# bkomuves/zikkurat-algebra

Hardware: AMD Instinct MI355X
Metric: BLS12-381 G1 MSM pairs/sec at 2^20; Fr NTT 2^24 elems/sec (1/2/4/8 GPU) (higher is better)
Workload: dtype u32-limb Montgomery Fp (381-bit)

## Files before the change

zikkurat-algebra_amd/csrc/zk_hostpool.cpp:

```cpp
#include <atomic>
#include <condition_variable>
#include <functional>
#include <memory>
#include <mutex>
#include <thread>
#include <vector>
#include "zk_hostpool.hpp"

namespace zk {

namespace {
struct Job {
  const std::function<void(int)> *fn;
  int n;
  std::atomic<int> next{0}, done{0};
  Job(const std::function<void(int)> *f, int count) : fn(f), n(count) {}
  bool has_work() const { return next.load(std::memory_order_relaxed) < n; }
  void drain() {
    for (;;) {
      const int i = next.fetch_add(1);
      if (i >= n) break;
      (*fn)(i);
      done.fetch_add(1, std::memory_order_release);
    }
  }
};

struct HostPool {
  std::mutex mu;
  std::condition_variable cv;
  std::vector<std::shared_ptr<Job>> active;
  int workers = 0;
  HostPool() {
    unsigned hw = std::thread::hardware_concurrency();
    workers = hw > 2 ? (int)(hw - 1 < 7 ? hw - 1 : 7) : 0;
    for (int i = 0; i < workers; i++) std::thread([this] { loop(); }).detach();
  }
  std::shared_ptr<Job> pick() {
    for (auto &j : active)
      if (j->has_work()) return j;
    return nullptr;
  }
  void loop() {
    for (;;) {
      std::shared_ptr<Job> job;
      {
        std::unique_lock<std::mutex> lk(mu);
        cv.wait(lk, [&] { return (job = pick()) != nullptr; });
      }
      job->drain();
    }
  }
  void run(int count, const std::function<void(int)> &f, const std::function<void()> *main_fn = nullptr) {
    auto job = std::make_shared<Job>(&f, count);
    {
      std::lock_guard<std::mutex> lk(mu);
      active.push_back(job);
    }
    cv.notify_all();
    if (main_fn) (*main_fn)();
    job->drain();
    while (job->done.load(std::memory_order_acquire) < count) std::this_thread::yield();
    std::lock_guard<std::mutex> lk(mu);
    for (size_t i = 0; i < active.size(); i++)
      if (active[i] == job) {
        active.erase(active.begin() + i);
        break;
      }
  }
};
}

static HostPool *shared_pool() {
  static HostPool *pool = new HostPool();
  return pool;
}

void host_parallel_for(int n, const std::function<void(int)> &fn) {
  if (n <= 0) return;
  HostPool *pool = shared_pool();
  if (n == 1 || pool->workers == 0) {
    for (int i = 0; i < n; i++) fn(i);
    return;
  }
  pool->run(n, fn);
}

void host_parallel_for_main(int n, const std::function<void(int)> &fn, const std::function<void()> &main_fn) {
  HostPool *pool = shared_pool();
  if (n <= 0 || pool->workers == 0) {
    for (int i = 0; i < n; i++) fn(i);
    main_fn();
    return;
  }
  pool->run(n, fn, &main_fn);
}

}
```

zikkurat-algebra_amd/csrc/zk_hostpool.hpp:

```cpp
#pragma once
#include <functional>

namespace zk {

void host_parallel_for(int n, const std::function<void(int)> &fn);

void host_parallel_for_main(int n, const std::function<void(int)> &fn, const std::function<void()> &main_fn);

}
```

zikkurat-algebra_amd/csrc/zk_msm_impl.hpp:

```cpp
#pragma once
#include <hipcub/hipcub.hpp>
#include <algorithm>
#include <atomic>
#include <chrono>
#include <memory>
#include <thread>
#include <vector>
#include "zk_curve.hpp"
#include "zk_quad.hpp"
#include "zk_host.hpp"
#include "zk_runtime.hpp"
#include "zk_msm.hpp"
#include "zk_ntt.hpp"

namespace zk {

template <class C>
__global__ void __launch_bounds__(256) k_points_int(const uint64_t *__restrict__ pts, int n,
                                                    uint32_t *__restrict__ out) {
  using F = typename C::Fp;
  constexpr int IN4 = 2 * F::N64 * 8 / 16;
  constexpr int OUT4 = aff_words<F>() / 4;
  constexpr int ST4 = IN4 > OUT4 ? IN4 : OUT4;
  __shared__ uint4 stage[256 * ST4];
// ... 473 lines not shown
        if (first_run && bbeg < cs) {
          xyzz_store(ivals + (size_t)(2 * t) * xyzz_words<F>(), acc);
          k0 = b;
        } else {
          xyzz_store(buckets + (size_t)b * xyzz_words<F>(), acc);
        }
        first_run = false;
        do {
          b++;
          bbeg = bend;
          bend = bnext;
          bnext = offsets[min(b + 2, nb)];
        } while (bend <= e);
        start_run(b);
      }
      if (P.x.v[0] != 0xffffffffu) {
        if (c0 & 0x80000000u) {
          Fe<F> ny;
          fe_neg(ny, P.y);
          P.y = ny;
        }
        xyzz_acc_aff(acc, P);
      }
      c0 = c1;
      c1 = c2;
    }
    const bool lpart = bbeg < cs, rpart = bend > ce;
    if (rpart && !(first_run && lpart)) {
      tail_b = b;
      tail_slot = first_run ? 2 * t : 2 * t + 1;
    } else if (lpart || rpart) {
      xyzz_store(ivals + (size_t)(2 * t) * xyzz_words<F>(), acc);
      k0 = b;
    } else {
      xyzz_store(buckets + (size_t)b * xyzz_words<F>(), acc);
    }
    head_end = k0 != nb && !(first_run && rpart);
    asm volatile("s_waitcnt vmcnt(0)" ::: "memory");
  }
  __builtin_amdgcn_fence(__ATOMIC_RELEASE, "workgroup");
  const uint32_t nhead = (uint32_t)__shfl_down((int)(head_end ? k0 : nb), 1, 64);
  const bool merge = tail_b != nb && lane < 63 && nhead == tail_b;
  if (__any(merge)) {
    __builtin_amdgcn_fence(__ATOMIC_ACQUIRE, "workgroup");
    if (merge) {
      const uint32_t *src = ivals + (size_t)(2 * t + 2) * xyzz_words<F>();
      uint32_t wds[xyzz_words<F>()];
#pragma unroll
      for (int i = 0; i < xyzz_words<F>(); i++) wds[i] = __hip_atomic_load(src + i, __ATOMIC_RELAXED, __HIP_MEMORY_SCOPE_AGENT);
      Xyzz<F> o;
      xyzz_load(o, wds);
      xyzz_add(acc, o);
    }
  }
  if (tail_b != nb) {
    if (merge) {
      xyzz_store(buckets + (size_t)tail_b * xyzz_words<F>(), acc);
    } else {
      xyzz_store(ivals + (size_t)tail_slot * xyzz_words<F>(), acc);
      if (tail_slot == 2 * t) k0 = tail_b; else k1 = tail_b;
    }
  }
  if (__shfl_up((int)merge, 1, 64) && lane > 0) k0 = nb;
  if (2 * t < nslots) {
    ikeys[2 * t] = k0;
    ikeys[2 * t + 1] = k1;
  }
}

static __global__ void __launch_bounds__(256) k_fill_mark(const uint32_t *__restrict__ off, uint32_t nb, int first,
                                                          uint8_t *__restrict__ filled) {
  const uint32_t b = blockIdx.x * blockDim.x + threadIdx.x;
  if (b >= nb) return;
  const uint8_t f = off[b + 1] > off[b] ? 1 : 0;
  filled[b] = first ? f : (uint8_t)(filled[b] | f);
}

static __global__ void __launch_bounds__(256) k_item_flags(const uint32_t *__restrict__ ikeys, const uint32_t *__restrict__ count,
                                                    uint32_t nslots_max, uint32_t nb, uint32_t *__restrict__ flags) {
  const uint32_t i = blockIdx.x * blockDim.x + threadIdx.x;
  if (i >= nslots_max) return;
  const uint32_t n = count ? *count : nslots_max;
  flags[i] = (i < n && ikeys[i] < nb) ? 1u : 0u;
}
#ifndef ZK_STITCH_RAW
#define ZK_STITCH_RAW 1
#endif
template <class C, int BS>
__global__ void __launch_bounds__(BS) k_stitch_blk(const uint32_t *__restrict__ keys, const uint32_t *__restrict__ idx,
                                                   const uint32_t *__restrict__ vals,
                                                   const uint32_t *__restrict__ count, uint32_t nb, uint32_t W,
                                                   uint32_t B, uint32_t *__restrict__ buckets,
                                                   uint32_t *__restrict__ okeys, uint32_t *__restrict__ ovals,
                                                   uint32_t nout) {
  using F = typename C::Fp;
  constexpr int XW = xyzz_words<F>();
  __shared__ uint4 stitch_lds4[BS * XW / 4];
  uint32_t *lv = reinterpret_cast<uint32_t *>(stitch_lds4);
  __shared__ uint32_t skey[BS];
  const uint32_t M = *count;
  const uint32_t t = threadIdx.x, blk = blockIdx.x;
  const uint32_t base = blk * BS;
  if (base >= M) {
    if (t < 2 && 2 * blk + t < nout) okeys[2 * blk + t] = nb;
    return;
  }
  const uint32_t nv = min((uint32_t)BS, M - base);
  const uint32_t j = base + t;
  const bool valid = t < nv;
  const uint32_t key = valid ? keys[j] : 0xffffffffu;
  skey[t] = key;
  Xyzz<F> acc;
  if (valid) xyzz_load(acc, vals + (size_t)idx[j] * XW);
  else xyzz_set_inf(acc);
  __syncthreads();
  for (uint32_t d = 1; d < nv; d <<= 1) {
    const bool need = valid && t >= d && skey[t - d] == key;
    if (!__syncthreads_or(need)) break;
    xyzz_store(lv + (size_t)t * XW, acc);
    __syncthreads();
    if (need) {
      Xyzz<F> o;
      xyzz_load(o, lv + (size_t)(t - d) * XW);
      xyzz_add_red(acc, o);
    }
    __syncthreads();
  }
  if (!valid) return;
  const bool seg_last = t == nv - 1 || skey[t + 1] != key;
  if (!seg_last) return;
  const bool touches_start = skey[0] == key;
  const bool touches_end = t == nv - 1;
  const bool cont_in = touches_start && base > 0 && keys[base - 1] == key;
  const bool cont_out = touches_end && base + nv < M && keys[base + nv] == key;
  if (!cont_in && !cont_out) {
    xyzz_store(buckets + (size_t)key * XW, acc);
  } else {
    xyzz_store(ovals + (size_t)(touches_start ? 2 * blk : 2 * blk + 1) * XW, acc);
  }
  const uint32_t item_key = (cont_in || cont_out) ? key : nb;
  if (touches_start) okeys[2 * blk] = item_key;
  if (touches_end) okeys[2 * blk + 1] = touches_start ? nb : item_key;
}

#ifndef ZK_STITCH_QUAD
#define ZK_STITCH_QUAD 1
#endif
constexpr int STITCH_QBS = 64;
template <class C>
__global__ void __launch_bounds__(256) k_stitch_blk_q(const uint32_t *__restrict__ keys, const uint32_t *__restrict__ idx,
                                                      const uint32_t *__restrict__ vals,
                                                      const uint32_t *__restrict__ count, uint32_t nb,
                                                      uint32_t *__restrict__ buckets, uint32_t *__restrict__ okeys,
                                                      uint32_t *__restrict__ ovals, uint32_t nout) {
  using F = typename C::Fp;
  constexpr int XW = xyzz_words<F>();
  constexpr uint32_t BSQ = STITCH_QBS;
  __shared__ uint4 item_lds4[BSQ * XW / 4];
  __shared__ uint32_t skey[BSQ];
  uint32_t *lv = reinterpret_cast<uint32_t *>(item_lds4);
  uint32_t *const park = nullptr;
  const uint32_t M = *count;
  const uint32_t tq = threadIdx.x >> 2, q = threadIdx.x & 3, blk = blockIdx.x;
  const uint32_t base = blk * BSQ;
  if (base >= M) {
    if (threadIdx.x < 2 && 2 * blk + threadIdx.x < nout) okeys[2 * blk + threadIdx.x] = nb;
// ... 728 lines not shown
    add(maxent * 2);
    add((s.nmat2() + 1) * 4 * 2);
  }
  add(s.NS * (nb + 1) * 4);
  add(nb);
  add(ns0 * (xw + 4) + ns0 * 16 + 64);
  add(ns1 * (xw + 4) * 2);
  add(nb * xw);
  add((size_t)s.W * s.NY * xw);
  add(cub > cub2 ? cub : cub2);
  if (s.NS > 1) add(cub > cub2 ? cub : cub2);
  return bytes + (1 << 20);
}

inline std::atomic<int> &msm_last_groups() {
  static std::atomic<int> v{0};
  return v;
}

inline std::atomic<int> &msm_profile_flag() {
  static std::atomic<int> on{0};
  return on;
}
struct PhaseProf {
  bool on = false;
  hipStream_t st = nullptr;
  std::vector<std::pair<const char *, hipEvent_t>> ev;
  explicit PhaseProf(hipStream_t s) : st(s) {
    on = msm_profile_flag().load() != 0;
    mark("start");
  }
  void mark(const char *name) {
    if (!on) return;
    hipEvent_t e;
    ZK_CHECK(hipEventCreate(&e));
    ZK_CHECK(hipEventRecord(e, st));
    ev.emplace_back(name, e);
  }
  void report(double host_ms) {
    if (!on) return;
    ZK_CHECK(hipStreamSynchronize(st));
    fprintf(stderr, "[zk msm]");
    for (size_t i = 1; i < ev.size(); i++) {
      float ms = 0;
      ZK_CHECK(hipEventElapsedTime(&ms, ev[i - 1].second, ev[i].second));
      fprintf(stderr, " %s=%.3f", ev[i].first, ms);
    }
    fprintf(stderr, " host_finish=%.3f ms\n", host_ms);
    for (auto &e : ev) ZK_CHECK(hipEventDestroy(e.second));
    ev.clear();
  }
};

struct ScalarSlice {
  const uint64_t *data;
  int stride, loff, nread;
  bool mont;
};

template <class C>
struct GroupPass {
  using F = typename C::Fp;
  static constexpr int STITCH_BS = stitch_bs<F>();
  Device &dev;
  MsmShape s;
  ScalarSlice sc;
  int wbase, timer_slot;
  const uint32_t *pts_int;
  uint64_t *h;
  PhaseProf *prof;
  hipStream_t st;
  size_t nb, xw, maxent, ns0, ns1, cub = 0;
  uint32_t *list, *dig, *tmpv, *cnt, *coff, *offsets, *ikeys0, *ivals0, *ckeys, *cidx, *flags, *pos, *ccount;
  uint16_t *tmpf, *tmpf2 = nullptr;
  uint32_t *cnt2 = nullptr, *coff2 = nullptr;
  uint32_t *okA, *ovA, *okB, *ovB, *buckets, *Y;
  void *cubtmp;
  uint8_t *filled = nullptr;
  hipStream_t sst = nullptr;
  void *cubtmp_sort = nullptr;
  const uint64_t *pts_ref = nullptr;
  std::vector<hipEvent_t> sorted_ev;
  hipEvent_t presorted = nullptr;
  const uint32_t *inK, *inV;
  size_t slots;
  uint32_t *outK, *outV, *altK, *altV;

  GroupPass(Device &d, const MsmShape &shape, const ScalarSlice &scal, int wb, const uint32_t *pts, uint64_t *hh,
            PhaseProf *pr, hipStream_t stream, int tslot)
      : dev(d), s(shape), sc(scal), wbase(wb), timer_slot(tslot), pts_int(pts), h(hh), prof(pr), st(stream) {
    const int n = s.n;
    nb = (size_t)s.W * s.B;
    xw = xyzz_words<F>();
    maxent = (size_t)s.W * n;
    ZK_REQUIRE(maxent <= MSM_MAX_PASS_ENTRIES, "msm: window group exceeds the sort capacity (internal sizing bug)");
    list = dev.arena.take<uint32_t>(maxent);
    dig = dev.arena.take<uint32_t>(maxent);
    tmpv = dev.arena.take<uint32_t>(maxent);
    tmpf = dev.arena.take<uint16_t>(maxent);
    cnt = dev.arena.take<uint32_t>(s.nmat() + 1);
    coff = dev.arena.take<uint32_t>(s.nmat() + 1);
    if (s.s2) {
      tmpf2 = dev.arena.take<uint16_t>(maxent);
      cnt2 = dev.arena.take<uint32_t>(s.nmat2() + 1);
      coff2 = dev.arena.take<uint32_t>(s.nmat2() + 1);
    }
    offsets = dev.arena.take<uint32_t>((size_t)s.NS * (nb + 1));
    if (s.NS > 1) filled = dev.arena.take<uint8_t>(nb);
    ns0 = stitch_slots0(s);
    ns1 = stitch_slots1(s, stitch_bs0<F>());
    ikeys0 = dev.arena.take<uint32_t>(ns0);
    ivals0 = dev.arena.take<uint32_t>(ns0 * xw);
    ckeys = dev.arena.take<uint32_t>(ns0);
    cidx = dev.arena.take<uint32_t>(ns0);
    flags = dev.arena.take<uint32_t>(ns0);
    pos = dev.arena.take<uint32_t>(ns0);
    ccount = dev.arena.take<uint32_t>(16);
    okA = dev.arena.take<uint32_t>(ns1);
    ovA = dev.arena.take<uint32_t>(ns1 * xw);
    okB = dev.arena.take<uint32_t>(ns1);
    ovB = dev.arena.take<uint32_t>(ns1 * xw);
    buckets = dev.arena.take<uint32_t>(nb * xw);
    Y = dev.arena.take<uint32_t>((size_t)s.W * s.NY * xw);
    size_t cub2 = 0;
    ZK_CHECK(hipcub::DeviceScan::ExclusiveSum(nullptr, cub, cnt, coff, (int)(s.nmat() + 1), st));
    ZK_CHECK(hipcub::DeviceScan::ExclusiveSum(nullptr, cub2, flags, pos, (int)ns0, st));
    if (cub2 > cub) cub = cub2;
    if (s.s2) {
      size_t cub3 = 0;
      ZK_CHECK(hipcub::DeviceScan::ExclusiveSum(nullptr, cub3, cnt2, coff2, (int)(s.nmat2() + 1), st));
      if (cub3 > cub) cub = cub3;
    }
    cubtmp = dev.arena.take<char>(cub);
    if (s.NS > 1) cubtmp_sort = dev.arena.take<char>(cub);
  }
  void mark(const char *what) {
    if (prof && wbase == 0) prof->mark(what);
  }

  void sort(int sp, hipStream_t st, void *cubtmp) {
    const int n = s.n, c = s.c;
    const int lo = s.split_lo(sp), hi = s.split_lo(sp + 1);
    const uint32_t base = (uint32_t)((size_t)s.W * lo);
    hipLaunchKernelGGL(k_digits<C>, dim3(div_up(hi - lo, 256)), dim3(256), 0, st, sc.data, n, lo, hi, sc.stride,
                       sc.loff, sc.nread, sc.mont ? 1 : 0, c, wbase, s.W, dig);
    ZK_CHECK(hipGetLastError());
    if (st == this->st) mark("digits");
    const dim3 grid((unsigned)s.nwg, (unsigned)s.W);
    hipLaunchKernelGGL(k_coarse<false>, grid, dim3(256), 0, st, dig, n, lo, hi, s.M, s.fs, s.nbins, cnt, tmpv + base,
                       tmpf + base);
    ZK_CHECK(hipGetLastError());
    size_t cb = cub;
    ZK_CHECK(hipcub::DeviceScan::ExclusiveSum(cubtmp, cb, cnt, coff, (int)(s.nmat() + 1), st));
    hipLaunchKernelGGL(k_coarse<true>, grid, dim3(256), 0, st, dig, n, lo, hi, s.M, s.fs, s.nbins, coff, tmpv + base,
                       tmpf + base);
    ZK_CHECK(hipGetLastError());
    const uint32_t *fv = tmpv + base, *fcoff = coff;
    const uint16_t *ff = tmpf + base;
    int fnwg = s.nwg, fs = s.fs;
    uint32_t nq = (uint32_t)(s.W * s.nbins);
    if (s.s2) {
      const int nsub = 1 << s.s2, s2sh = s.fs - s.s2;
      const dim3 g2((unsigned)s.nwg2, nq);
      hipLaunchKernelGGL(k_split<false>, g2, dim3(256), 0, st, coff, s.nwg, s2sh, nsub, cnt2, tmpv + base, tmpf + base,
                         dig + base, tmpf2 + base);
      ZK_CHECK(hipGetLastError());
      size_t cb2 = cub;
      ZK_CHECK(hipcub::DeviceScan::ExclusiveSum(cubtmp, cb2, cnt2, coff2, (int)(s.nmat2() + 1), st));
      hipLaunchKernelGGL(k_split<true>, g2, dim3(256), 0, st, coff, s.nwg, s2sh, nsub, coff2, tmpv + base, tmpf + base,
                         dig + base, tmpf2 + base);
      ZK_CHECK(hipGetLastError());
      fv = dig + base;
      ff = tmpf2 + base;
      fcoff = coff2;
      fnwg = s.nwg2;
      fs = s2sh;
      nq *= (uint32_t)nsub;
    }
    const int cap = fine_stage_cap(fs);
    const int lds = (4 << fs) + 4 * cap;
    if ((size_t)(hi - lo) * s.W >= (size_t)nq * 4096) {
      ZK_CHECK(hipFuncSetAttribute((const void *)k_fine<1024, 4, true>, hipFuncAttributeMaxDynamicSharedMemorySize,
                                   lds));
      hipLaunchKernelGGL((k_fine<1024, 4, true>), dim3(nq), dim3(1024), lds, st, fcoff, fnwg, nq, fs, cap, fv, ff,
                         list + base, offsets + (size_t)sp * (nb + 1), base);
    } else {
      ZK_CHECK(hipFuncSetAttribute((const void *)k_fine<256, 1, false>, hipFuncAttributeMaxDynamicSharedMemorySize,
                                   lds));
      hipLaunchKernelGGL((k_fine<256, 1, false>), dim3(nq), dim3(256), lds, st, fcoff, fnwg, nq, fs, cap, fv, ff,
                         list + base, offsets + (size_t)sp * (nb + 1), base);
    }
    ZK_CHECK(hipGetLastError());
    if (st == this->st) mark("sort");
  }

  std::vector<hipEvent_t> wait_sc, wait_pt;
  const std::atomic<int> *ready_sc = nullptr, *ready_pt = nullptr;
  void wait_for(hipStream_t on, const std::vector<hipEvent_t> &ev, const std::atomic<int> *ready, int sp) {
    if (sp >= (int)ev.size() || !ev[sp]) return;
    if (ready)
      while (!ready[sp].load(std::memory_order_acquire)) std::this_thread::yield();
    ZK_CHECK(hipStreamWaitEvent(on, ev[sp], 0));
  }
  void convert(int sp) {
    const int lo = s.split_lo(sp), hi = s.split_lo(sp + 1);
    if (hi <= lo) return;
    hipLaunchKernelGGL(k_points_int<C>, dim3(div_up(hi - lo, 256)), dim3(256), 0, st,
                       pts_ref + (size_t)lo * 2 * C::NP64, hi - lo, const_cast<uint32_t *>(pts_int) + (size_t)lo * aff_words<F>());
    ZK_CHECK(hipGetLastError());
  }
  int ch0 = 0;
  void accumulate(int sp) {
    if (sp == 0) timer_begin(dev, timer_slot, st);
    const size_t npts = (size_t)s.split_lo(sp + 1) - (size_t)s.split_lo(sp);
    const int CH = s.split_ch(sp);
    ch0 = CH;
    const size_t nsl = 2 * (((size_t)s.W * npts + CH - 1) / CH);
    hipLaunchKernelGGL(k_accum<C>, dim3(div_up(nsl / 2, 256)), dim3(256), 0, st, pts_int, list,
                       offsets + (size_t)sp * (nb + 1), (uint32_t)nb, CH, (uint32_t)s.W, (uint32_t)s.B, buckets,
                       ikeys0, ivals0, (uint32_t)nsl, (const uint8_t *)(sp > 0 ? filled : nullptr));
    ZK_CHECK(hipGetLastError());
    if (sp == s.NS - 1) timer_end(dev, timer_slot, st);
    mark("accum");
    inK = ikeys0;
    inV = ivals0;
    slots = nsl;
    level = 0;
    outK = okA; outV = ovA; altK = okB; altV = ovB;
  }
  void fill_mark(int sp) {
    hipLaunchKernelGGL(k_fill_mark, dim3(div_up(nb, 256)), dim3(256), 0, st, offsets + (size_t)sp * (nb + 1),
                       (uint32_t)nb, sp == 0 ? 1 : 0, filled);
    ZK_CHECK(hipGetLastError());
  }

  int level = 0;
  bool stitch_level() {
    const bool raw = ZK_STITCH_RAW && level++ > 0;
    const bool quad0 = stitch_bs0<F>() == STITCH_QBS && (ns0 <= 65536 || ch0 >= 64);
    const int bs = raw ? STITCH_BS : (quad0 ? STITCH_QBS : STITCH_BS);
    const bool final_level = slots <= (size_t)bs;
    const size_t nout = final_level ? 2 : 2 * ((slots + bs - 1) / bs);
    if (raw) {
      hipLaunchKernelGGL((k_stitch_raw<C, STITCH_BS>), dim3((unsigned)((slots + STITCH_BS - 1) / STITCH_BS)),
                         dim3(STITCH_BS), 0, st, inK, inV, (uint32_t)slots, (uint32_t)nb, final_level ? 1 : 0,
                         buckets, outK, outV);
      ZK_CHECK(hipGetLastError());
    } else {
      hipLaunchKernelGGL(k_item_flags, dim3(div_up(slots, 256)), dim3(256), 0, st, inK, (const uint32_t *)nullptr,
                         (uint32_t)slots, (uint32_t)nb, flags);
      ZK_CHECK(hipGetLastError());
      size_t cb = cub;
      ZK_CHECK(hipcub::DeviceScan::ExclusiveSum(cubtmp, cb, flags, pos, (int)slots, st));
      hipLaunchKernelGGL(k_item_index, dim3(div_up(slots, 256)), dim3(256), 0, st, inK, flags, pos, (uint32_t)slots,
                         ckeys, cidx, ccount);
      ZK_CHECK(hipGetLastError());
      bool launched = false;
      if constexpr (stitch_bs0<F>() == STITCH_QBS) {
        if (quad0) {
          hipLaunchKernelGGL(k_stitch_blk_q<C>, dim3((unsigned)(nout / 2)), dim3(256), 0, st, ckeys, cidx, inV, ccount,
                             (uint32_t)nb, buckets, outK, outV, (uint32_t)nout);
          launched = true;
        }
      }
      if (!launched)
        hipLaunchKernelGGL((k_stitch_blk<C, STITCH_BS>), dim3((unsigned)(nout / 2)), dim3(STITCH_BS), 0, st, ckeys,
                           cidx, inV, ccount, (uint32_t)nb, (uint32_t)s.W, (uint32_t)s.B, buckets, outK, outV,
                           (uint32_t)nout);
      ZK_CHECK(hipGetLastError());
    }
    inK = outK; inV = outV; slots = nout;
    uint32_t *tk = outK, *tv = outV;
    outK = altK; outV = altV; altK = tk; altV = tv;
    return final_level;
  }

  void reduce_tail() {
    const int c = s.c;
    const int n0 = s.r0.count * s.r0.G, n1 = s.r1.count * s.r1.G;
    if (n0 % 256 == 0 && n1 % 256 == 0) {
      const unsigned nblk = (unsigned)(s.W * (n0 + n1) / 256);
      bool two_waves = false;
      if constexpr (is_base_field<F>()) {
        two_waves = ysum3_on((size_t)nblk * 256);
        if (two_waves)
          hipLaunchKernelGGL((k_ysum3<C>), dim3(nblk), dim3(256), 0, st, buckets, offsets, (const uint8_t *)filled,
                             s.W, c, s.l0, s.r0, s.r1, Y);
      } else if (ysum_g2_lds<F>()) {
        two_waves = true;
        hipLaunchKernelGGL((k_ysum3<C, 1>), dim3(nblk), dim3(256), 0, st, buckets, offsets, (const uint8_t *)filled,
                           s.W, c, s.l0, s.r0, s.r1, Y);
      }
      if (!two_waves)
        hipLaunchKernelGGL((k_ysum2<C, is_base_field<F>() ? ZK_YSUM_PF != 0 : ZK_YSUM_PF_G2 != 0>), dim3(nblk),
                           dim3(256), 0, st, buckets, offsets,
                           (const uint8_t *)filled, s.W, c, s.l0, s.r0, s.r1, Y);
    } else {
      const size_t lanes = (size_t)s.W * s.ylanes;
      hipLaunchKernelGGL(k_ysum<C>, dim3(div_up(lanes, 256)), dim3(256), 0, st, buckets, offsets,
                         (const uint8_t *)filled, s.W, c, s.l0, s.r0, s.r1, s.ylanes, Y);
    }
    ZK_CHECK(hipGetLastError());
    mark("ysum");
    hipLaunchKernelGGL(k_jobsum_blk<C>, dim3((unsigned)(s.W * c)), dim3(256), 0, st, Y, c, s.l0, h);
    ZK_CHECK(hipGetLastError());
    mark("jobsum");
  }

  void launch() {
    for (int sp = 0; sp < s.NS; sp++) {
      if (presorted) {
        ZK_CHECK(hipStreamWaitEvent(st, presorted, 0));
      } else if (sst) {
        wait_for(sst, wait_sc, ready_sc, sp);
        sort(sp, sst, cubtmp_sort);
        ZK_CHECK(hipEventRecord(sorted_ev[sp], sst));
      } else {
        wait_for(st, wait_sc, ready_sc, sp);
        sort(sp, st, cubtmp);
      }
      wait_for(st, wait_pt, ready_pt, sp);
      if (pts_ref) convert(sp);
      if (sst) ZK_CHECK(hipStreamWaitEvent(st, sorted_ev[sp], 0));
      accumulate(sp);
      for (bool final_level = false; !final_level;) final_level = stitch_level();
      if (s.NS > 1) fill_mark(sp);
    }
    mark("stitch");
    reduce_tail();
  }
  void finish() {
    stream_wait(dev, st);
    mark("export");
  }
};

template <class C>
static void finish_host(int c, int W, const uint64_t *exported, zkh::Xyzz<typename HostOf<C>::Fp> &out,
                        int bits = 0) {
  using HF = typename HostOf<C>::Fp;
  const int NP = C::NP64;
  const int J = c, E = bits ? c : c - 1;
  std::vector<zkh::Jac<HF>> V(W);
  std::unique_ptr<std::atomic<int>[]> ready(new std::atomic<int>[W]);
  for (int w = 0; w < W; w++) ready[w].store(0, std::memory_order_relaxed);
  std::atomic<int> next_win{0};
  auto window = [&](int i) {
    const int w = W - 1 - i;
    std::vector<zkh::Xyzz<HF>> Z(E);
    for (auto &z : Z) zkh::xyzz_set_inf(z);
    for (int j = 0; j < J; j++) {
      if (bits && c * w + j >= bits) break;
      const uint64_t *q = exported + ((size_t)w * J + j) * 4 * NP;
      zkh::Xyzz<HF> p;
      memcpy(p.X.v, q + 0 * NP, NP * 8);
      memcpy(p.Y.v, q + 1 * NP, NP * 8);
      memcpy(p.ZZ.v, q + 2 * NP, NP * 8);
      memcpy(p.ZZZ.v, q + 3 * NP, NP * 8);
      if (zkh::xyzz_is_inf(p)) continue;
      const int e = bits ? j : (j == 0 ? 0 : j - 1);
      zkh::xyzz_add(Z[e], Z[e], p);
    }
    zkh::Xyzz<HF> acc;
    zkh::xyzz_set_inf(acc);
    for (int e = E - 1; e >= 0; e--) {
      zkh::xyzz_dbl(acc, acc);
      zkh::xyzz_add(acc, acc, Z[e]);
    }
    zkh::xyzz_to_jac(V[w], acc);
    ready[w].store(1, std::memory_order_release);
  };
  zkh::Jac<HF> acc;
  zkh::jac_set_inf(acc);
  auto claim = [&]() -> bool {
    const int i = next_win.fetch_add(1);
    if (i >= W) return false;
    window(i);
    return true;
  };
  auto chain = [&] {
    for (int w = W - 1; w >= 0; w--) {
      for (int k = 0; k < c; k++) zkh::jac_dbl(acc, acc);
      while (!ready[w].load(std::memory_order_acquire))
        if (!claim()) std::this_thread::yield();
      zkh::jac_add(acc, acc, V[w]);
    }
  };
  const int nthreads = W < 8 ? W : 8;
  host_parallel_for_main(nthreads, [&](int) { while (claim()) {} }, chain);
  zkh::jac_to_xyzz(out, acc);
}

#ifndef ZK_MSM_BITS_MAX
#define ZK_MSM_BITS_MAX 4096
#endif
inline int msm_bits_max() {
  static const int v = [] {
    const char *e = getenv("ZK_MSM_BITS_MAX");
    return e ? atoi(e) : ZK_MSM_BITS_MAX;
  }();
  return v;
}
inline int msm_bits_groups(int n) {
  static const int g = [] {
    const char *e = getenv("ZK_MSM_BITS_G");
    const int v = e ? atoi(e) : 256;
    return v >= 1 ? v : 256;
  }();
  int K = (n + g - 1) / g;
  if (K > BITACC_MAX_K) K = BITACC_MAX_K;
  return (n + K - 1) / K;
}

template <class C>
static void msm_run_bits(Device &dev, int n, const ScalarSlice &sc_in, const uint64_t *points, bool host_inputs,
                         int nbits, zkh::Xyzz<typename HostOf<C>::Fp> &out) {
  using F = typename C::Fp;
  constexpr int XW = xyzz_words<F>();
  ZK_REQUIRE(nbits >= 1 && nbits <= 256, "msm: bit-job path takes at most 256-bit scalars (internal)");
  const int G = msm_bits_groups(n), K = (n + G - 1) / G;
  ZK_REQUIRE(K >= 1 && K <= BITACC_MAX_K, "msm: bit-job chunk larger than k_bitacc's LDS staging (internal)");
  hipStream_t st = dev.stream;
  const size_t sc_bytes = host_inputs ? (size_t)n * sc_in.stride * 8 : 0;
  const size_t pt_bytes = host_inputs ? (size_t)n * 2 * C::NP64 * 8 : 0;
  const size_t int_bytes = (size_t)n * aff_words<F>() * 4;
  const size_t part_bytes = (size_t)nbits * G * XW * 4;
  const size_t exp_bytes = (size_t)nbits * 4 * C::NP64 * 8;
  const size_t need = sc_bytes + pt_bytes + int_bytes + part_bytes + 4 * 256;
  if (!dev.arena.try_reserve(need)) {
    ZK_CHECK(hipStreamSynchronize(st));
    ntt_release(dev);
    ZK_REQUIRE(dev.arena.try_reserve(need), "msm: out of device memory");
  }
  dev.arena.reset();
  msm_last_groups().store(1);
  PhaseProf prof(st);
  ScalarSlice sc = sc_in;
  const uint64_t *pts_ref = points;
  if (host_inputs) {
    uint64_t *a = dev.arena.take<uint64_t>((size_t)n * sc_in.stride);
    uint64_t *b = dev.arena.take<uint64_t>((size_t)n * 2 * C::NP64);
    ZK_CHECK(hipMemcpyAsync(a, sc_in.data, sc_bytes, hipMemcpyHostToDevice, st));
    ZK_CHECK(hipMemcpyAsync(b, points, pt_bytes, hipMemcpyHostToDevice, st));
    sc.data = a;
    pts_ref = b;
  }
  uint32_t *pts_int = dev.arena.take<uint32_t>((size_t)n * aff_words<F>());
  uint32_t *part = dev.arena.take<uint32_t>((size_t)nbits * G * XW);
  uint64_t *h = reinterpret_cast<uint64_t *>(dev.host_staging(exp_bytes + 64));
  hipLaunchKernelGGL(k_points_int<C>, dim3(div_up(n, 256)), dim3(256), 0, st, pts_ref, n, pts_int);
  ZK_CHECK(hipGetLastError());
  prof.mark("points");
  timer_begin(dev, 0, st);
  hipLaunchKernelGGL(k_bitacc<C>, dim3((unsigned)G), dim3(256), 0, st, sc.data, n, sc.stride, sc.loff, sc.nread,
                     sc.mont ? 1 : 0, nbits, K, pts_int, part);
  ZK_CHECK(hipGetLastError());
  timer_end(dev, 0, st);
  prof.mark("bitacc");
  hipLaunchKernelGGL(k_bitsum<C>, dim3((unsigned)nbits), dim3(256), 0, st, part, G, h);
  ZK_CHECK(hipGetLastError());
  prof.mark("bitsum");
  stream_wait(dev, st);
  prof.mark("export");
  timer_collect(dev);
  const auto t0 = std::chrono::steady_clock::now();
  constexpr int BW = 8;
  finish_host<C>(BW, (nbits + BW - 1) / BW, h, out, nbits);
// ... 51 lines not shown
                                           group_bytes<C>(make_shape(n, c, W - Wa, 1)));
  while (!ahead && !dev.arena.try_reserve(sc_bytes + pt_bytes + int_bytes + 3 * 256 + group_bytes<C>(s))) {
    if (!dropped_twiddles) {
      ZK_CHECK(hipStreamSynchronize(st));
      ntt_release(dev);
      dropped_twiddles = true;
      continue;
    }
    ZK_REQUIRE(Wg > 1, "msm: out of device memory (one window per pass does not fit)");
    Wg = (Wg + 1) / 2;
    s = make_shape(n, c, Wg, splits(Wg));
  }
  const int NS = s.NS;
  msm_last_groups().store(ahead ? 2 : (W + Wg - 1) / Wg);
  dev.arena.reset();
  ScalarSlice sc = sc_in;
  uint32_t *pts_int = nullptr;
  PhaseProf prof(st);
  bool inputs_on_aux = false;
  std::atomic<int> ready_sc[ZK_MSM_SPLITS_MAX], ready_pt[ZK_MSM_SPLITS_MAX];
  std::string copy_err;
  std::mutex copy_mu;
  std::vector<std::thread> copier_v;
  JoinAll join_copier{copier_v};
  uint64_t *pts_ref = nullptr;
  if (host_inputs) {
    uint64_t *a = dev.arena.take<uint64_t>((size_t)n * sc_in.stride);
    uint64_t *b = dev.arena.take<uint64_t>((size_t)n * 2 * C::NP64);
    pts_int = dev.arena.take<uint32_t>((size_t)n * aff_words<F>());
    sc.data = a;
    pts_ref = b;
    hipStream_t st2 = dev.aux_stream();
    for (int h = 0; h < 3 * NS; h++) dev.split_event(h);
    for (int h = 0; h < NS; h++) {
      ready_sc[h].store(0, std::memory_order_relaxed);
      ready_pt[h].store(0, std::memory_order_relaxed);
    }
    const int stride = sc_in.stride;
    const uint64_t *sc_host = sc_in.data;
    const MsmShape shp = s;
    copier_v.emplace_back([&dev, st2, NS, shp, a, b, stride, sc_host, points, &ready_sc, &ready_pt, &copy_err,
                           &copy_mu] {
      catch_into(&copy_err, &copy_mu, [&] {
      ZK_CHECK(hipSetDevice(dev.id));
      for (int h = 0; h < NS; h++) {
        const int lo = shp.split_lo(h), hi = shp.split_lo(h + 1);
        ZK_CHECK(hipMemcpyAsync(a + (size_t)lo * stride, sc_host + (size_t)lo * stride,
                                (size_t)(hi - lo) * stride * 8, hipMemcpyHostToDevice, st2));
        ZK_CHECK(hipEventRecord(dev.split_event(3 * h), st2));
        ready_sc[h].store(1, std::memory_order_release);
        const size_t off = (size_t)lo * 2 * C::NP64;
        ZK_CHECK(hipMemcpyAsync(b + off, points + off, (size_t)(hi - lo) * 2 * C::NP64 * 8, hipMemcpyHostToDevice, st2));
        ZK_CHECK(hipEventRecord(dev.split_event(3 * h + 1), st2));
        ready_pt[h].store(1, std::memory_order_release);
      }
      });
      for (int h = 0; h < NS; h++) {
        ready_sc[h].store(1, std::memory_order_release);
        ready_pt[h].store(1, std::memory_order_release);
      }
    });
    inputs_on_aux = true;
  } else {
    pts_int = dev.arena.take<uint32_t>((size_t)n * aff_words<F>());
    if (ahead) ZK_CHECK(hipEventRecord(dev.split_event(0), st));
    hipLaunchKernelGGL(k_points_int<C>, dim3(div_up(n, 256)), dim3(256), 0, st, points, n, pts_int);
    ZK_CHECK(hipGetLastError());
  }
  prof.mark("points");
  const size_t mark = dev.arena.used();
  const size_t per_w = (size_t)c * 4 * C::NP64;
  uint64_t *h = reinterpret_cast<uint64_t *>(dev.host_staging((size_t)W * per_w * 8 + 64));
  if (ahead) {
    GroupPass<C> pa(dev, make_shape(n, c, Wa, 1), sc, 0, pts_int, h, &prof, st, 0);
    GroupPass<C> pb(dev, make_shape(n, c, W - Wa, 1), sc, Wa, pts_int, h + (size_t)Wa * per_w, &prof, st, 1);
    hipStream_t sst = dev.aux2_stream();
    ZK_CHECK(hipStreamWaitEvent(sst, dev.split_event(0), 0));
    pa.sort(0, sst, pa.cubtmp);
    ZK_CHECK(hipEventRecord(dev.split_event(1), sst));
    pb.sort(0, sst, pb.cubtmp);
    ZK_CHECK(hipEventRecord(dev.split_event(2), sst));
    pa.presorted = dev.split_event(1);
    pb.presorted = dev.split_event(2);
    pa.launch();
    pb.launch();
    pb.finish();
    timer_collect(dev);
    const auto t0 = std::chrono::steady_clock::now();
    finish_host<C>(c, W, h, out);
    prof.report(std::chrono::duration<double, std::milli>(std::chrono::steady_clock::now() - t0).count());
    return;
  }
  for (int wbase = 0; wbase < W; wbase += Wg) {
    dev.arena.rewind(mark);
    const MsmShape sg = (wbase + Wg <= W) ? s : make_shape(n, c, W - wbase);
    GroupPass<C> pass(dev, sg, sc, wbase, pts_int, h + (size_t)wbase * per_w, &prof, st, wbase == 0 ? 0 : -1);
    if (inputs_on_aux) {
      ZK_REQUIRE(sg.NS == NS, "msm: split pipeline shape mismatch (internal)");
      for (int h = 0; h < NS; h++) {
        pass.wait_sc.push_back(dev.split_event(3 * h));
        pass.wait_pt.push_back(dev.split_event(3 * h + 1));
        pass.sorted_ev.push_back(dev.split_event(3 * h + 2));
      }
      pass.ready_sc = ready_sc;
      pass.ready_pt = ready_pt;
      pass.pts_ref = pts_ref;
      static const bool sort_inline = [] {
        const char *e = getenv("ZK_MSM_SORT_INLINE");
        return e && e[0] == '1';
      }();
      if (NS > 1 && !sort_inline) pass.sst = dev.aux2_stream();
    }
    inputs_on_aux = false;
    pass.launch();
    for (auto &t : copier_v)
      if (t.joinable()) t.join();
    pass.finish();
    rethrow_first(copy_err);
  }
  timer_collect(dev);
  const auto t0 = std::chrono::steady_clock::now();
  finish_host<C>(c, W, h, out);
  prof.report(std::chrono::duration<double, std::milli>(std::chrono::steady_clock::now() - t0).count());
}


template <class C>
size_t msm_workspace_bytes(int n, int nl, bool mont, bool host_inputs, int window, int groups) {
  using F = typename C::Fp;
  if (n <= 0) return 0;
  const int nread = nl < 4 ? nl : 4;
  const int nbits = mont ? HostOf<C>::Fr::BITS : 64 * nread;
  if (!(window >= 4 && window <= 24) && n <= msm_bits_max()) {
    const size_t io = host_inputs ? (size_t)n * nl * 8 + (size_t)n * 2 * C::NP64 * 8 : 0;
    return io + (size_t)n * aff_words<F>() * 4 + (size_t)nbits * msm_bits_groups(n) * xyzz_words<F>() * 4 + 4 * 256;
  }
  const int c = (window >= 4 && window <= 24)
                    ? window
                    : (is_base_field<F>() ? msm_default_window_bits(n, nbits) : msm_default_window(n));
  const int W = nbits / c + 1;
  const int g = groups < 1 ? 1 : (groups > W ? W : groups);
  const int Wg = (W + g - 1) / g;
  const size_t sc_bytes = host_inputs ? (size_t)n * nl * 8 : 0;
  const size_t pt_bytes = host_inputs ? (size_t)n * 2 * C::NP64 * 8 : 0;
  const size_t int_bytes = (size_t)n * aff_words<F>() * 4;
  const int NS = msm_splits(n, host_inputs, Wg == W);
  if (msm_ahead<C>(n, host_inputs, W, Wg)) {
    const int Wa = (W + 1) / 2;
    return int_bytes + 3 * 256 + group_bytes<C>(make_shape(n, c, Wa, 1)) + group_bytes<C>(make_shape(n, c, W - Wa, 1));
  }
  return sc_bytes + pt_bytes + int_bytes + 3 * 256 + group_bytes<C>(make_shape(n, c, Wg, NS));
}

template <class C>
static void msm_xyzz(Device &dev, int n, const uint64_t *scalars, int nl, const uint64_t *points, bool host_inputs,
                     bool mont, int window, zkh::Xyzz<typename HostOf<C>::Fp> &acc) {
  using HF = typename HostOf<C>::Fp;
  if (mont || nl <= 4) {
    msm_run<C>(dev, n, ScalarSlice{scalars, nl, 0, nl < 4 ? nl : 4, mont}, points, host_inputs, window, acc);
  } else {
    zkh::xyzz_set_inf(acc);
    const int nsl = (nl + 3) / 4;
    for (int j = nsl - 1; j >= 0; j--) {
      for (int k = 0; k < 256; k++) zkh::xyzz_dbl(acc, acc);
      const int nread = nl - 4 * j < 4 ? nl - 4 * j : 4;
      zkh::Xyzz<HF> r;
      msm_run<C>(dev, n, ScalarSlice{scalars, nl, 4 * j, nread, false}, points, host_inputs, window, r);
      zkh::xyzz_add(acc, acc, r);
    }
  }
}

template <class C>
void msm_g1(int n, const uint64_t *scalars, int nl, const uint64_t *points, bool host_inputs, bool mont,
            int window, uint64_t *out_proj) {
  using HF = typename HostOf<C>::Fp;
  ZK_REQUIRE(nl >= 1, "msm: expo_nlimbs must be >= 1");
  zkh::Xyzz<HF> acc;
  const std::vector<int> set = host_inputs ? device_set() : std::vector<int>();
  const int G = (int)set.size();
  if (G > 1 && n > 0) {
    std::vector<zkh::Xyzz<HF>> part(G);
    std::vector<std::thread> th;
    std::string err;
    std::mutex emu;
    {
    JoinAll join_all{th};
    for (int k = 0; k < G; k++) {
      const size_t lo = (size_t)n * k / G, hi = (size_t)n * (k + 1) / G;
      int slot = 0;
      for (int j = 0; j < k; j++) slot += set[j] == set[k];
      zkh::xyzz_set_inf(part[k]);
      if (hi == lo) continue;
      th.emplace_back([&, k, lo, hi, slot] {
        catch_into(&err, &emu, [&] {
          ZK_CHECK(hipSetDevice(set[k]));
// ... 30 lines not shown
```

zikkurat-algebra_amd/csrc/zk_runtime.cpp:

```cpp
#include "zk_runtime.hpp"
#include <atomic>
#include <chrono>
#include <map>
#include <algorithm>
#include <cstring>
#include <thread>

namespace zk {

static std::atomic<int> g_error_mode{0};
void set_error_mode(int mode) { g_error_mode.store(mode == 1 ? 1 : 0); }

[[noreturn]] void fatal(const char *what, const char *file, int line) {
  char msg[512];
  snprintf(msg, sizeof msg, "%s (%s:%d)", what, file, line);
  fprintf(stderr, "[zkalgebra_gpu] %s: %s\n", g_error_mode.load() ? "error" : "fatal", msg);
  fflush(stderr);
  if (g_error_mode.load()) throw Error(msg);
  abort();
}

static thread_local std::string t_last_error;
void record_error(const char *msg) { t_last_error = msg; }
int take_last_error(char *msg, size_t cap) {
// ... 95 lines not shown

Device &device_context(int id, int slot) {
  std::lock_guard<std::mutex> lock(g_devices_mu);
  auto it = g_devices.find({id, slot});
  if (it != g_devices.end()) return *it->second;
  DeviceGuard on(id);
  hipStream_t stream = nullptr;
  ZK_CHECK(hipStreamCreateWithFlags(&stream, hipStreamNonBlocking));
  Device *d = new Device();
  d->id = id;
  d->slot = slot;
  d->uid = (int)g_devices.size();
  d->stream = stream;
  g_devices[{id, slot}] = d;
  return *d;
}

Device &current_device() {
  int id = 0;
  ZK_CHECK(hipGetDevice(&id));
  return device_context(id, 0);
}

std::vector<Device *> all_devices() {
  std::lock_guard<std::mutex> lock(g_devices_mu);
  std::vector<Device *> v;
  for (auto &kv : g_devices) v.push_back(kv.second);
  return v;
}

static std::mutex g_set_mu;
static std::vector<int> g_set;
static bool g_set_init = false;

static int device_count_or_zero() {
  int n = 0;
  if (hipGetDeviceCount(&n) != hipSuccess) {
    (void)hipGetLastError();
    return 0;
  }
  return n;
}

std::vector<int> device_set() {
  std::lock_guard<std::mutex> lock(g_set_mu);
  if (!g_set_init) {
    g_set_init = true;
    const char *env = getenv("ZKG_DEVICES");
    if (env && *env) {
      const int count = device_count_or_zero();
      std::vector<int> v;
      if (std::string(env) == "all") {
        for (int i = 0; i < count; i++) v.push_back(i);
      } else {
        const char *p = env;
        while (*p) {
          char *end = nullptr;
          const long id = strtol(p, &end, 10);
          if (end == p || id < 0 || id >= count) {
            fprintf(stderr, "[zkalgebra_gpu] ZKG_DEVICES=%s: invalid device list, ignored\n", env);
            v.clear();
            break;
          }
          v.push_back((int)id);
          p = *end == ',' ? end + 1 : end;
        }
      }
      g_set = v;
    }
  }
  return g_set;
}

int set_device_set(const int *ids, int n) {
  const int count = device_count_or_zero();
  for (int i = 0; i < n; i++)
    if (ids[i] < 0 || ids[i] >= count) return -1;
  std::lock_guard<std::mutex> lock(g_set_mu);
  g_set.assign(ids, ids + (n > 0 ? n : 0));
  g_set_init = true;
  return 0;
}

void stream_wait(Device &dev, hipStream_t st) {
  if (!dev.sync_ev) ZK_CHECK(hipEventCreateWithFlags(&dev.sync_ev, hipEventDisableTiming));
  ZK_CHECK(hipEventRecord(dev.sync_ev, st));
  const auto t0 = std::chrono::steady_clock::now();
  for (;;) {
    const hipError_t e = hipEventQuery(dev.sync_ev);
    if (e == hipSuccess) return;
    if (e != hipErrorNotReady) ZK_CHECK(e);
    const double us = std::chrono::duration<double, std::micro>(std::chrono::steady_clock::now() - t0).count();
    if (us > 20000) std::this_thread::sleep_for(std::chrono::microseconds(20));
    else if (us > 200) std::this_thread::yield();
  }
}

static std::atomic<bool> g_timer_on{false};

void timer_set_enabled(bool on) { g_timer_on.store(on); }

void timer_begin(Device &dev, int slot, hipStream_t st) {
  if (slot < 0 || slot > 1) return;
  if (!g_timer_on.load()) {
    dev.timer.armed[slot] = false;
    return;
  }
  if (!dev.timer.ev0[slot]) {
    ZK_CHECK(hipEventCreate(&dev.timer.ev0[slot]));
    ZK_CHECK(hipEventCreate(&dev.timer.ev1[slot]));
  }
  dev.timer.armed[slot] = true;
  dev.timer.counted = true;
  ZK_CHECK(hipEventRecord(dev.timer.ev0[slot], st ? st : dev.stream));
}

void timer_end(Device &dev, int slot, hipStream_t st) {
  if (slot < 0 || slot > 1) return;
  if (dev.timer.armed[slot]) ZK_CHECK(hipEventRecord(dev.timer.ev1[slot], st ? st : dev.stream));
}

void timer_collect(Device &dev) {
  for (int k = 0; k < 2; k++) {
    if (!dev.timer.armed[k]) continue;
    float ms = 0;
    ZK_CHECK(hipEventSynchronize(dev.timer.ev1[k]));
    ZK_CHECK(hipEventElapsedTime(&ms, dev.timer.ev0[k], dev.timer.ev1[k]));
    dev.timer.total_ms += ms;
    dev.timer.armed[k] = false;
  }
  if (dev.timer.counted) dev.timer.launches++;
  dev.timer.counted = false;
}

void timer_reset_all() {
  const std::vector<Device *> devs = all_devices();
  for (Device *d : devs)
    if (d) {
      std::lock_guard<std::mutex> lock(d->mu);
      d->timer.total_ms = 0;
      d->timer.launches = 0;
    }
}

void timer_read_all(double *total_ms, long *launches) {
  const std::vector<Device *> devs = all_devices();
  double t = 0;
  long n = 0;
  for (Device *d : devs)
    if (d) {
      std::lock_guard<std::mutex> lock(d->mu);
      t += d->timer.total_ms;
      n += d->timer.launches;
    }
  if (total_ms) *total_ms = t;
  if (launches) *launches = n;
}


void copy_to_host(Device &dev, hipStream_t st, void *dst, const void *src, size_t bytes) {
  constexpr size_t PIECE = (size_t)32 << 20;
  constexpr int THREADS = 8;
  if (bytes < 2 * PIECE) {
    ZK_CHECK(hipMemcpyAsync(dst, src, bytes, hipMemcpyDeviceToHost, st));
    stream_wait(dev, st);
    return;
  }
  if (dev.xfer_cap < 2 * PIECE) {
    if (dev.xfer) ZK_CHECK(hipHostFree(dev.xfer));
    dev.xfer = nullptr;
    ZK_CHECK(hipHostMalloc(&dev.xfer, 2 * PIECE, hipHostMallocDefault));
    dev.xfer_cap = 2 * PIECE;
  }
  for (int j = 0; j < 2; j++)
// ... 35 lines not shown
```

zikkurat-algebra_amd/csrc/zk_runtime.hpp:

```cpp
#pragma once
#include <hip/hip_runtime.h>
#include <stdint.h>
#include <stdio.h>
#include <stdlib.h>
#include <atomic>
#include <functional>
#include <memory>
#include <mutex>
#include <stdexcept>
#include <string>
#include <thread>
#include <vector>
#include "zk_hostpool.hpp"

namespace zk {

struct Error : std::runtime_error {
  using std::runtime_error::runtime_error;
};
[[noreturn]] void fatal(const char *what, const char *file, int line);
void set_error_mode(int mode);
void record_error(const char *msg);
int take_last_error(char *msg, size_t cap);
template <class Fn>
// ... 30 lines not shown
  ~JoinAll() {
    for (auto &t : th)
      if (t.joinable()) t.join();
  }
};
#define ZK_CHECK(x)                                                       \
  do {                                                                    \
    hipError_t e__ = (x);                                                 \
    if (e__ != hipSuccess) {                                              \
      (void)hipGetLastError();  \
      ::zk::fatal(hipGetErrorString(e__), __FILE__, __LINE__);            \
    }                                                                     \
  } while (0)
#define ZK_REQUIRE(cond, msg)                                             \
  do {                                                                    \
    if (!(cond)) ::zk::fatal(msg, __FILE__, __LINE__);                    \
  } while (0)

struct DeviceGuard {
  int prev = -1;
  explicit DeviceGuard(int dev) {
    ZK_CHECK(hipGetDevice(&prev));
    if (prev != dev) ZK_CHECK(hipSetDevice(dev));
  }
  DeviceGuard(const DeviceGuard &) = delete;
  DeviceGuard &operator=(const DeviceGuard &) = delete;
  ~DeviceGuard() {
    int cur = -1;
    if (hipGetDevice(&cur) != hipSuccess || cur != prev)
      if (hipSetDevice(prev) != hipSuccess) (void)hipGetLastError();
  }
};

class Arena {
 public:
  void reserve(size_t bytes);
  bool try_reserve(size_t bytes);
  void release();
  size_t capacity() const { return cap_; }
  void reset() { off_ = 0; }
  void rewind(size_t off) { off_ = off; }
  template <class T>
  T *take(size_t count) {
    size_t bytes = (count * sizeof(T) + 255) & ~size_t(255);
    ZK_REQUIRE(off_ + bytes <= cap_, "zk arena overflow (internal sizing bug)");
    T *p = reinterpret_cast<T *>(base_ + off_);
    off_ += bytes;
    return p;
  }
  size_t used() const { return off_; }
  ~Arena();

 private:
  char *base_ = nullptr;
  size_t cap_ = 0;
  size_t off_ = 0;
};

struct KernelTimer {
  hipEvent_t ev0[2] = {nullptr, nullptr}, ev1[2] = {nullptr, nullptr};
  bool armed[2] = {false, false};
  bool counted = false;
  double total_ms = 0;
  long launches = 0;
};

void arena_set_limit(size_t bytes);

struct Device {
  int id = 0;
  int slot = 0;
  int uid = 0;
  hipStream_t stream = nullptr;
  Arena arena;
  std::mutex mu;
  void *pinned = nullptr;
  size_t pinned_cap = 0;
  void *host_staging(size_t bytes);
  void *xfer = nullptr;
  size_t xfer_cap = 0;
  hipEvent_t xfer_ev[2] = {nullptr, nullptr};
  KernelTimer timer;
  hipEvent_t sync_ev = nullptr;
  hipStream_t aux = nullptr;
  hipEvent_t aux_ev = nullptr;
  hipStream_t aux_stream();
  hipStream_t aux2 = nullptr;
  hipStream_t aux2_stream();
  std::vector<hipEvent_t> split_ev;
  hipEvent_t split_event(int h);
  void release_memory();
};

void copy_to_host(Device &dev, hipStream_t st, void *dst, const void *src, size_t bytes);

void stream_wait(Device &dev, hipStream_t st);

Device &current_device();
Device &device_context(int id, int slot);
std::vector<Device *> all_devices();

std::vector<int> device_set();
int set_device_set(const int *ids, int n);

void timer_set_enabled(bool on);
void timer_begin(Device &dev, int slot = 0, hipStream_t st = nullptr);
void timer_end(Device &dev, int slot = 0, hipStream_t st = nullptr);
void timer_collect(Device &dev);
void timer_reset_all();
void timer_read_all(double *total_ms, long *launches);

inline unsigned div_up(size_t a, size_t b) { return (unsigned)((a + b - 1) / b); }

}
```

Baseline: 332.4 million.

## Warm host pool early, spin-wait in chain, and replace scan-based item compaction

Replaces the flags/scan/index item compaction with a two-kernel tile count-and-place compaction, cutting launches and the hipcub scan. An early event is recorded before the final jobsum kernel. When the host sync loop sees that event complete, it wakes the host thread pool into a short busy-spin window so workers are hot for the CPU-side window reduction. The host chain loop now spins before yielding and only claims work when windows remain. These trade CPU busy-spinning for lower wake-up latency. The serial prefix sum inside each place block adds cost when there are many tiles.

New measurement: 333.8 million (median of 6 runs). No clear change (+0.4%).

```diff
diff --git a/zikkurat-algebra_amd/csrc/zk_hostpool.cpp b/zikkurat-algebra_amd/csrc/zk_hostpool.cpp
--- a/zikkurat-algebra_amd/csrc/zk_hostpool.cpp
+++ b/zikkurat-algebra_amd/csrc/zk_hostpool.cpp
@@ -1,5 +1,7 @@
 #include <atomic>
+#include <chrono>
 #include <condition_variable>
+#include <cstdint>
 #include <functional>
 #include <memory>
 #include <mutex>
@@ -31,6 +33,20 @@
   std::condition_variable cv;
   std::vector<std::shared_ptr<Job>> active;
   int workers = 0;
+  std::atomic<int64_t> hot_until{0};
+  std::atomic<uint64_t> published{0};
+  static int64_t now_ns() {
+    return std::chrono::duration_cast<std::chrono::nanoseconds>(std::chrono::steady_clock::now().time_since_epoch())
+        .count();
+  }
+  bool hot() const { return now_ns() < hot_until.load(std::memory_order_acquire); }
+  void expect() {
+    {
+      std::lock_guard<std::mutex> lk(mu);
+      hot_until.store(now_ns() + 1000000, std::memory_order_release);
+    }
+    cv.notify_all();
+  }
   HostPool() {
     unsigned hw = std::thread::hardware_concurrency();
     workers = hw > 2 ? (int)(hw - 1 < 7 ? hw - 1 : 7) : 0;
@@ -44,9 +60,15 @@
   void loop() {
     for (;;) {
       std::shared_ptr<Job> job;
+      uint64_t seen = 0;
       {
         std::unique_lock<std::mutex> lk(mu);
-        cv.wait(lk, [&] { return (job = pick()) != nullptr; });
+        cv.wait(lk, [&] { return (job = pick()) != nullptr || hot(); });
+        seen = published.load(std::memory_order_relaxed);
+      }
+      if (!job) {
+        while (published.load(std::memory_order_acquire) == seen && hot()) {}
+        continue;
       }
       job->drain();
     }
@@ -56,6 +78,8 @@
     {
       std::lock_guard<std::mutex> lk(mu);
       active.push_back(job);
+      hot_until.store(0, std::memory_order_release);
+      published.fetch_add(1, std::memory_order_release);
     }
     cv.notify_all();
     if (main_fn) (*main_fn)();
@@ -96,4 +120,9 @@
   pool->run(n, fn, &main_fn);
 }
 
+void host_pool_expect() {
+  HostPool *pool = shared_pool();
+  if (pool->workers > 0) pool->expect();
 }
+
+}
diff --git a/zikkurat-algebra_amd/csrc/zk_hostpool.hpp b/zikkurat-algebra_amd/csrc/zk_hostpool.hpp
--- a/zikkurat-algebra_amd/csrc/zk_hostpool.hpp
+++ b/zikkurat-algebra_amd/csrc/zk_hostpool.hpp
@@ -7,4 +7,6 @@
 
 void host_parallel_for_main(int n, const std::function<void(int)> &fn, const std::function<void()> &main_fn);
 
+void host_pool_expect();
+
 }
diff --git a/zikkurat-algebra_amd/csrc/zk_msm_impl.hpp b/zikkurat-algebra_amd/csrc/zk_msm_impl.hpp
--- a/zikkurat-algebra_amd/csrc/zk_msm_impl.hpp
+++ b/zikkurat-algebra_amd/csrc/zk_msm_impl.hpp
@@ -579,6 +579,58 @@
   if (i >= nslots_max) return;
   const uint32_t n = count ? *count : nslots_max;
   flags[i] = (i < n && ikeys[i] < nb) ? 1u : 0u;
+}
+#ifndef ZK_ITEM_COMPACT2
+#define ZK_ITEM_COMPACT2 1
+#endif
+constexpr uint32_t ITEM_TILES_MAX = 2048;
+static __global__ void __launch_bounds__(256) k_item_count(const uint32_t *__restrict__ ikeys, uint32_t nslots,
+                                                           uint32_t nb, uint32_t tile, uint32_t *__restrict__ tcnt) {
+  __shared__ uint32_t wsum[4];
+  const uint32_t t = threadIdx.x, lane = t & 63, wave = t >> 6;
+  const uint32_t lo = blockIdx.x * tile, hi = min(nslots, lo + tile);
+  uint32_t cnt = 0;
+  for (uint32_t i = lo + t; i < hi; i += 256) cnt += ikeys[i] < nb ? 1u : 0u;
+  for (int o = 32; o >= 1; o >>= 1) cnt += (uint32_t)__shfl_down((int)cnt, o);
+  if (lane == 0) wsum[wave] = cnt;
+  __syncthreads();
+  if (t == 0) tcnt[blockIdx.x] = wsum[0] + wsum[1] + wsum[2] + wsum[3];
+}
+static __global__ void __launch_bounds__(256) k_item_place(const uint32_t *__restrict__ ikeys,
+                                                           const uint32_t *__restrict__ tcnt, uint32_t nslots,
+                                                           uint32_t nb, uint32_t tile, uint32_t *__restrict__ okeys,
+                                                           uint32_t *__restrict__ oidx, uint32_t *__restrict__ ocount) {
+  __shared__ uint32_t wsum[4];
+  const uint32_t t = threadIdx.x, lane = t & 63, wave = t >> 6, blk = blockIdx.x;
+  uint32_t before = 0;
+  for (uint32_t b = t; b < blk; b += 256) before += tcnt[b];
+  for (int o = 32; o >= 1; o >>= 1) before += (uint32_t)__shfl_down((int)before, o);
+  if (lane == 0) wsum[wave] = before;
+  __syncthreads();
+  uint32_t base = wsum[0] + wsum[1] + wsum[2] + wsum[3];
+  const uint32_t lo = blk * tile, hi = min(nslots, lo + tile);
+  for (uint32_t i0 = lo; i0 < hi; i0 += 256) {
+    const uint32_t i = i0 + t;
+    const uint32_t k = i < hi ? ikeys[i] : nb;
+    const bool v = k < nb;
+    const uint64_t bal = __ballot(v);
+    __syncthreads();
+    if (lane == 0) wsum[wave] = (uint32_t)__popcll(bal);
+    __syncthreads();
+    uint32_t off = 0, tot = 0;
+#pragma unroll
+    for (uint32_t w = 0; w < 4; w++) {
+      off += w < wave ? wsum[w] : 0u;
+      tot += wsum[w];
+    }
+    if (v) {
+      const uint32_t o = base + off + (uint32_t)__popcll(bal & ((1ull << lane) - 1));
+      okeys[o] = k;
+      oidx[o] = i;
+    }
+    base += tot;
+  }
+  if (blk == gridDim.x - 1 && t == 0) *ocount = base;
 }
 #ifndef ZK_STITCH_RAW
 #define ZK_STITCH_RAW 1
@@ -1473,6 +1525,7 @@
   const uint64_t *pts_ref = nullptr;
   std::vector<hipEvent_t> sorted_ev;
   hipEvent_t presorted = nullptr;
+  bool last_pass = false;
   const uint32_t *inK, *inV;
   size_t slots;
   uint32_t *outK, *outV, *altK, *altV;
@@ -1638,6 +1691,15 @@
                          buckets, outK, outV);
       ZK_CHECK(hipGetLastError());
     } else {
+#if ZK_ITEM_COMPACT2
+      const uint32_t tile = 256 * (uint32_t)((slots + 256 * (size_t)ITEM_TILES_MAX - 1) / (256 * (size_t)ITEM_TILES_MAX));
+      const unsigned ntiles = (unsigned)((slots + tile - 1) / tile);
+      hipLaunchKernelGGL(k_item_count, dim3(ntiles), dim3(256), 0, st, inK, (uint32_t)slots, (uint32_t)nb, tile, flags);
+      ZK_CHECK(hipGetLastError());
+      hipLaunchKernelGGL(k_item_place, dim3(ntiles), dim3(256), 0, st, inK, (const uint32_t *)flags, (uint32_t)slots,
+                         (uint32_t)nb, tile, ckeys, cidx, ccount);
+      ZK_CHECK(hipGetLastError());
+#else
       hipLaunchKernelGGL(k_item_flags, dim3(div_up(slots, 256)), dim3(256), 0, st, inK, (const uint32_t *)nullptr,
                          (uint32_t)slots, (uint32_t)nb, flags);
       ZK_CHECK(hipGetLastError());
@@ -1646,6 +1708,7 @@
       hipLaunchKernelGGL(k_item_index, dim3(div_up(slots, 256)), dim3(256), 0, st, inK, flags, pos, (uint32_t)slots,
                          ckeys, cidx, ccount);
       ZK_CHECK(hipGetLastError());
+#endif
       bool launched = false;
       if constexpr (stitch_bs0<F>() == STITCH_QBS) {
         if (quad0) {
@@ -1693,6 +1756,7 @@
     }
     ZK_CHECK(hipGetLastError());
     mark("ysum");
+    if (last_pass) ZK_CHECK(hipEventRecord(dev.early_event(), st));
     hipLaunchKernelGGL(k_jobsum_blk<C>, dim3((unsigned)(s.W * c)), dim3(256), 0, st, Y, c, s.l0, h);
     ZK_CHECK(hipGetLastError());
     mark("jobsum");
@@ -1721,7 +1785,7 @@
     reduce_tail();
   }
   void finish() {
-    stream_wait(dev, st);
+    stream_wait(dev, st, last_pass ? dev.early_event() : nullptr);
     mark("export");
   }
 };
@@ -1772,8 +1836,10 @@
   auto chain = [&] {
     for (int w = W - 1; w >= 0; w--) {
       for (int k = 0; k < c; k++) zkh::jac_dbl(acc, acc);
-      while (!ready[w].load(std::memory_order_acquire))
-        if (!claim()) std::this_thread::yield();
+      for (int spins = 0; !ready[w].load(std::memory_order_acquire);) {
+        if (next_win.load(std::memory_order_relaxed) <= W - 1 - w) claim();
+        else if (++spins > 4096) std::this_thread::yield();
+      }
       zkh::jac_add(acc, acc, V[w]);
     }
   };
@@ -1991,6 +2057,7 @@
     ZK_CHECK(hipEventRecord(dev.split_event(2), sst));
     pa.presorted = dev.split_event(1);
     pb.presorted = dev.split_event(2);
+    pb.last_pass = true;
     pa.launch();
     pb.launch();
     pb.finish();
@@ -2021,6 +2088,7 @@
       if (NS > 1 && !sort_inline) pass.sst = dev.aux2_stream();
     }
     inputs_on_aux = false;
+    pass.last_pass = wbase + Wg >= W;
     pass.launch();
     for (auto &t : copier_v)
       if (t.joinable()) t.join();
diff --git a/zikkurat-algebra_amd/csrc/zk_runtime.cpp b/zikkurat-algebra_amd/csrc/zk_runtime.cpp
--- a/zikkurat-algebra_amd/csrc/zk_runtime.cpp
+++ b/zikkurat-algebra_amd/csrc/zk_runtime.cpp
@@ -201,7 +201,12 @@
   return 0;
 }
 
-void stream_wait(Device &dev, hipStream_t st) {
+hipEvent_t Device::early_event() {
+  if (!early_ev) ZK_CHECK(hipEventCreateWithFlags(&early_ev, hipEventDisableTiming));
+  return early_ev;
+}
+
+void stream_wait(Device &dev, hipStream_t st, hipEvent_t early) {
   if (!dev.sync_ev) ZK_CHECK(hipEventCreateWithFlags(&dev.sync_ev, hipEventDisableTiming));
   ZK_CHECK(hipEventRecord(dev.sync_ev, st));
   const auto t0 = std::chrono::steady_clock::now();
@@ -209,6 +214,15 @@
     const hipError_t e = hipEventQuery(dev.sync_ev);
     if (e == hipSuccess) return;
     if (e != hipErrorNotReady) ZK_CHECK(e);
+    if (early) {
+      const hipError_t ee = hipEventQuery(early);
+      if (ee == hipSuccess) {
+        host_pool_expect();
+        early = nullptr;
+      } else if (ee != hipErrorNotReady) {
+        ZK_CHECK(ee);
+      }
+    }
     const double us = std::chrono::duration<double, std::micro>(std::chrono::steady_clock::now() - t0).count();
     if (us > 20000) std::this_thread::sleep_for(std::chrono::microseconds(20));
     else if (us > 200) std::this_thread::yield();
diff --git a/zikkurat-algebra_amd/csrc/zk_runtime.hpp b/zikkurat-algebra_amd/csrc/zk_runtime.hpp
--- a/zikkurat-algebra_amd/csrc/zk_runtime.hpp
+++ b/zikkurat-algebra_amd/csrc/zk_runtime.hpp
@@ -136,6 +136,8 @@
   hipEvent_t xfer_ev[2] = {nullptr, nullptr};
   KernelTimer timer;
   hipEvent_t sync_ev = nullptr;
+  hipEvent_t early_ev = nullptr;
+  hipEvent_t early_event();
   hipStream_t aux = nullptr;
   hipEvent_t aux_ev = nullptr;
   hipStream_t aux_stream();
@@ -148,7 +150,7 @@
 
 void copy_to_host(Device &dev, hipStream_t st, void *dst, const void *src, size_t bytes);
 
-void stream_wait(Device &dev, hipStream_t st);
+void stream_wait(Device &dev, hipStream_t st, hipEvent_t early = nullptr);
 
 Device &current_device();
 Device &device_context(int id, int slot);
```
